# joyecnu/STTODE

Hardware: AMD Instinct MI355X
Metric: predicted-trajectories/sec (20-sample best-of-K) (higher is better)
Workload: dtype f32

## Files before the change

### sttode_amd/csrc/chain.hpp

```cpp
#pragma once
#include <hip/hip_runtime.h>

typedef float f32x4 __attribute__((ext_vector_type(4)));

#define STT_WAVE 64
#define STT_FENCE() asm volatile("" ::: "memory")

__device__ __forceinline__ f32x4 mfma_k16(f32x4 acc, const f32x4 w, const f32x4 b) {
    acc = __builtin_amdgcn_mfma_f32_16x16x4f32(w[0], b[0], acc, 0, 0, 0);
    acc = __builtin_amdgcn_mfma_f32_16x16x4f32(w[1], b[1], acc, 0, 0, 0);
    acc = __builtin_amdgcn_mfma_f32_16x16x4f32(w[2], b[2], acc, 0, 0, 0);
    acc = __builtin_amdgcn_mfma_f32_16x16x4f32(w[3], b[3], acc, 0, 0, 0);
    return acc;
}

__device__ __forceinline__ f32x4 ld4(const float* p) { return *reinterpret_cast<const f32x4*>(p); }
__device__ __forceinline__ void st4(float* p, const f32x4 v) { *reinterpret_cast<f32x4*>(p) = v; }

__device__ __forceinline__ f32x4 relu4(f32x4 v) {
    v[0] = fmaxf(v[0], 0.f); v[1] = fmaxf(v[1], 0.f); v[2] = fmaxf(v[2], 0.f); v[3] = fmaxf(v[3], 0.f);
    return v;
}

__device__ __forceinline__ float sigmoidf_(float x) {
    return __builtin_amdgcn_rcpf(1.0f + __builtin_amdgcn_exp2f(-1.4426950408889634f * x));
}
__device__ __forceinline__ float tanhf_(float x) {
    return 1.0f - 2.0f * __builtin_amdgcn_rcpf(1.0f + __builtin_amdgcn_exp2f(2.8853900817779268f * x));
}
__device__ __forceinline__ float sigmoid_prescaled(float t) { return __builtin_amdgcn_rcpf(1.0f + __builtin_amdgcn_exp2f(t)); }
__device__ __forceinline__ float tanh_prescaled(float t) { return fmaf(-2.0f, __builtin_amdgcn_rcpf(1.0f + __builtin_amdgcn_exp2f(t)), 1.0f); }

__device__ __forceinline__ f32x4 splat4(float v) { f32x4 r = {v, v, v, v}; return r; }

__device__ __forceinline__ float colsum_q(float v) {
    v += __shfl_xor(v, 16, 64);
    v += __shfl_xor(v, 32, 64);
    return v;
}

__device__ __forceinline__ void layernorm64(f32x4 (&x)[4], const float* __restrict__ gamma, const float* __restrict__ beta, int q) {
    float s = 0.f;
#pragma unroll
    for (int T = 0; T < 4; ++T) s += (x[T][0] + x[T][1]) + (x[T][2] + x[T][3]);
    const float mean = colsum_q(s) * (1.0f / 64.0f);
    float v = 0.f;
#pragma unroll
    for (int T = 0; T < 4; ++T)
#pragma unroll
        for (int r = 0; r < 4; ++r) { const float d = x[T][r] - mean; v += d * d; }
    const float rstd = 1.0f / sqrtf(colsum_q(v) * (1.0f / 64.0f) + 1e-5f);
#pragma unroll
    for (int T = 0; T < 4; ++T) {
        const f32x4 g = ld4(gamma + 16 * T + 4 * q), b = ld4(beta + 16 * T + 4 * q);
// ... 27 lines not shown
```

### sttode_amd/csrc/chain32.hip

```cpp
#include "chain.hpp"
#include "latency_bodies.hpp"
#include "frontend_body.hpp"
#include "api_util.hpp"
#include "../../include/sttode_hip.h"
#include <cstdlib>
#include <cstddef>

#ifdef C32_DIAG_TRACE
__shared__ long long g_tr_ph[4];
#define C32_TRACE_BEGIN() long long _tr_t0 = 0, _tr_c0 = 0; if (threadIdx.x == 0 && A.dbg) { _tr_t0 = __builtin_amdgcn_s_memrealtime(); _tr_c0 = __builtin_amdgcn_s_memtime(); }
#define C32_TRACE_END(kind) do { if (threadIdx.x == 0 && A.dbg) { \
        const long long _t1 = __builtin_amdgcn_s_memrealtime(); unsigned _hw, _xcc; \
        asm volatile("s_getreg_b32 %0, hwreg(HW_REG_HW_ID)" : "=s"(_hw)); asm volatile("s_getreg_b32 %0, hwreg(HW_REG_XCC_ID)" : "=s"(_xcc)); \
        const unsigned long long _r = atomicAdd((unsigned long long*)A.dbg, 1ull); if ((long long)_r >= A.dbg[1]) break;  \
        long long* _p = A.dbg + 8 + _r * 12; _p[0] = A.trace_tag; _p[1] = blockIdx.x; _p[2] = (kind); _p[3] = _tr_t0; _p[4] = _t1; _p[5] = _hw; _p[6] = _xcc; \
        _p[8] = g_tr_ph[0]; _p[9] = g_tr_ph[1]; _p[10] = g_tr_ph[2]; _p[7] = __builtin_amdgcn_s_memtime() - _tr_c0; _p[11] = g_tr_ph[3]; } } while (0)
#define C32_TRACE_PHASE(i) do { if (threadIdx.x == 0) g_tr_ph[i] = __builtin_amdgcn_s_memrealtime(); } while (0)
#else
#define C32_TRACE_PHASE(i) do { } while (0)
#define C32_TRACE_BEGIN() do { } while (0)
#define C32_TRACE_END(kind) do { } while (0)
#endif

#include "role_body.hpp"

typedef float f32x16 __attribute__((ext_vector_type(16)));

#ifdef C32_DIAG_NOGATES
#define C32_SIG(x) ((x) * 1e-3f)
#define C32_TANH(x) ((x) * 1e-3f)
#else
#define C32_SIG(x) sigmoid_prescaled(x)
#define C32_TANH(x) tanh_prescaled(x)
#endif

#define C32_TILE 256
#define C32_CMAX 3
#define C32_RING (2 * C32_CMAX * C32_TILE)
#define C32_SLOT 256

struct Role32Args {
    const f32x4* pool; const int2* prog; int prog_len; const float* consts;
    const float* enc_in; const int* last;
    const float* g_in; const float* attn; int ld_attn;
    const float* xpad; int ldx;
    float* pf; float* state0; float* A0x; float* A0y; float* A1y;
    int n, Tp, kte, nwg;
    float ode_time;
    int prio;
    int* counter;
    float* zgen; unsigned zkey0, zkey1; int K;
    const float* past; const int* scene_ptr; int S; float* scene_orig; int* agent_scene;
    float* enc_in_w; float* xpad_w; float* cur_w; float* orig_w; int* last_w;
    float* m_ade; float* m_fde;
};

// ... 14 lines not shown
    int nworkers;
    long long* dbg;
    int trace_tag;
    int xcd_map;
    RoleArgs R;
    Role32Args R32;
};

template <int NY> struct C32Const {
    static constexpr int b2x = 0, b3x = 256, b2y = 288, b3y = 544, gb = 544 + 32 * NY, cb = gb + 384, b2m = cb + 32,
                         b3m = b2m + 256, total = b3m + 32 * NY;
};

__device__ __forceinline__ f32x16 splat16(float v) {
    f32x16 r;
#pragma unroll
    for (int e = 0; e < 16; ++e) r[e] = v;
    return r;
}
__device__ __forceinline__ f32x16 relu16(f32x16 v) {
#pragma unroll
    for (int e = 0; e < 16; ++e) v[e] = fmaxf(v[e], 0.f);
    return v;
}
__device__ __forceinline__ f32x16 ldrows(const float* p, int h) {
    f32x16 r;
#pragma unroll
    for (int a = 0; a < 4; ++a) {
        const f32x4 v = ld4(p + 8 * a + 4 * h);
        r[4 * a + 0] = v[0]; r[4 * a + 1] = v[1]; r[4 * a + 2] = v[2]; r[4 * a + 3] = v[3];
    }
    return r;
}

typedef const __attribute__((address_space(4))) int KProg;

template <int BUF, bool GEN, bool DYN = false>
struct ChainStreamT {
    static constexpr int kBuf = BUF;
    static constexpr int kPieces = (BUF / 64 + 3) / 4, kPairs = (kPieces + 1) / 2;
    const char* pool; KProg* prog; f32x4* ring;
    unsigned ring_addr, loff;
    unsigned qoff, qend;
    int par, lane, wave;
    int2 ld_v, ld_w;
    bool fetched;
// ... 98 lines not shown
        __builtin_amdgcn_sched_barrier(0);
    }
};
typedef ChainStreamT<C32_CMAX * C32_TILE, false> ChainStream;

__device__ __forceinline__ void tile_mma(f32x16& acc, const f32x4* __restrict__ t, const f32x16& B) {
#pragma unroll
    for (int g = 0; g < 4; ++g) {
        const f32x4 a = t[g * 64];
#pragma unroll
        for (int r = 0; r < 4; ++r) acc = __builtin_amdgcn_mfma_f32_32x32x2f32(a[r], B[4 * g + r], acc, 0, 0, 0);
    }
}

__device__ __forceinline__ void gather_rows(const void* base, unsigned voff, unsigned slot_addr) {
    glds16_sv<0>(base, voff, slot_addr);
    glds16_sv<32>(base, voff, slot_addr + 1024);
    glds16_sv<64>(base, voff, slot_addr + 2048);
    glds16_sv<96>(base, voff, slot_addr + 3072);
}
__device__ __forceinline__ unsigned row_off(int row, int width, int h) { return (unsigned)row * (unsigned)(width * 4) + (unsigned)h * 16; }

struct Frag { f32x4 a[4]; };
__device__ __forceinline__ void ldfrag(Frag& f, const f32x4* __restrict__ t) {
#pragma unroll
    for (int g = 0; g < 4; ++g) f.a[g] = t[g * 64];
}
__device__ __forceinline__ void tile_mma2(f32x16& acc, const Frag& cur, const f32x16& B, Frag& nxt, const f32x4* __restrict__ tn) {
#pragma unroll
    for (int g = 0; g < 4; ++g) {
        if (g == 2 && tn) {
            ldfrag(nxt, tn);
            __builtin_amdgcn_sched_barrier(0);
        }
#pragma unroll
        for (int r = 0; r < 4; ++r) acc = __builtin_amdgcn_mfma_f32_32x32x2f32(cur.a[g][r], B[4 * g + r], acc, 0, 0, 0);
    }
}

template <class ST>
__device__ __forceinline__ void tile_mma2f(ST& st, f32x16& acc, const Frag& cur, const f32x16& B, Frag& nxt, const f32x4* __restrict__ tn, int nf = 1) {
#pragma unroll
    for (int g = 0; g < 4; ++g) {
        if (g == 2) {
            __builtin_amdgcn_sched_barrier(0);
            if (nf >= 1) st.fetch();
            if (nf >= 2) st.fetch_more();
            if (tn) ldfrag(nxt, tn);
            __builtin_amdgcn_sched_barrier(0);
        }
#pragma unroll
        for (int r = 0; r < 4; ++r) acc = __builtin_amdgcn_mfma_f32_32x32x2f32(cur.a[g][r], B[4 * g + r], acc, 0, 0, 0);
    }
}

template <int KH, class ST>
__device__ __forceinline__ void mlp_l12(ST& st, const f32x4* slot, const f32x4* zslot, const f32x16* Bh, const float* tab, unsigned aoff,
                                        const float* tab_next, unsigned aoff_next, f32x16 (&acc2)[8], int lane) {
    const unsigned slot_addr = __builtin_amdgcn_readfirstlane(lds_addr(slot));
    constexpr int KT1 = 1 + KH;
    static_assert((KT1 + 8) % 3 == 0, "hidden tile must be a whole number of chunks");
#pragma unroll
    for (int R = 0; R < 8; ++R) acc2[R] = splat16(0.f);
#pragma unroll 1
    for (int ht = 0; ht < 16; ++ht) {
        f32x16 h1, zb;
#pragma unroll
        for (int a = 0; a < 4; ++a) {
            const f32x4 v = slot[a * 64 + lane];
            h1[4 * a + 0] = v[0]; h1[4 * a + 1] = v[1]; h1[4 * a + 2] = v[2]; h1[4 * a + 3] = v[3];
        }
#pragma unroll
        for (int a = 0; a < 4; ++a) {
            const f32x4 v = zslot[a * 64 + lane];
            zb[4 * a + 0] = v[0]; zb[4 * a + 1] = v[1]; zb[4 * a + 2] = v[2]; zb[4 * a + 3] = v[3];
// ... 20 lines not shown
            const f32x4* tn = (i % 3 < 2) ? st.cur() + (i % 3 + 1) * C32_TILE : nullptr;
            if (i == 0) {
                tile_mma2f(st, h1, fr[i & 1], zb, fr[(i + 1) & 1], tn);
            } else if (i < KT1) {
                if (i % 3 == 0) tile_mma2f(st, h1, fr[i & 1], Bh[i - 1], fr[(i + 1) & 1], tn);
                else tile_mma2(h1, fr[i & 1], Bh[i - 1], fr[(i + 1) & 1], tn);
            } else {
                if (i == KT1) h1 = relu16(h1);
                if (i % 3 == 0) tile_mma2f(st, acc2[i - KT1], fr[i & 1], h1, fr[(i + 1) & 1], tn);
                else tile_mma2(acc2[i - KT1], fr[i & 1], h1, fr[(i + 1) & 1], tn);
            }
        }
        st.end();
    }
}

template <int NO, int NEXT = 0, class ST>
__device__ __forceinline__ void mlp_l3(ST& st, f32x16 (&acc2)[8], const float* __restrict__ b2, const float* __restrict__ b3,
                                       f32x16 (&out)[NO], int h) {
#pragma unroll
    for (int R = 0; R < 8; ++R) {
        STT_FENCE();
        const f32x16 b = ldrows(b2 + 32 * R, h);
        acc2[R] = relu16(acc2[R] + b);
        asm volatile("" : "+v"(acc2[R]));
    }
    STT_FENCE();
#pragma unroll
    for (int o = 0; o < NO; ++o) out[o] = ldrows(b3 + 32 * o, h);
    Frag fr[2];
#pragma unroll
    for (int i = 0; i < 8 * NO; ++i) {
        if (i % 3 == 0) {
            if (i > 0) st.end();
            ldfrag(fr[i & 1], st.cur());
            const int left = 8 * NO - (i + 3);
            st.begin(left >= 3 ? 3 : left > 0 ? left : NEXT);
        }
        const f32x4* tn = (i % 3 < 2 && i + 1 < 8 * NO) ? st.cur() + (i % 3 + 1) * C32_TILE : nullptr;
        if (i % 3 == 0) tile_mma2f(st, out[i / 8], fr[i & 1], acc2[i % 8], fr[(i + 1) & 1], tn);
        else tile_mma2(out[i / 8], fr[i & 1], acc2[i % 8], fr[(i + 1) & 1], tn);
    }
    st.end();
}

typedef __bf16 bf16x8 __attribute__((ext_vector_type(8)));
typedef __bf16 bf16x2 __attribute__((ext_vector_type(2)));
// ... 247 lines not shown
            if (g >= g0 && g <= g1) fa.a[g] = tc[g * 64];
        st.begin(3);
#pragma unroll
        for (int g = 0; g < 4; ++g)
            if (g >= g0 && g <= g1)
#pragma unroll
                for (int r = 0; r < 4; ++r) e = __builtin_amdgcn_mfma_f32_32x32x2f32(fa.a[g][r], d[4 * g + r], e, 0, 0, 0);
        __builtin_amdgcn_sched_barrier(0);
        if (pre) st.take_prefetched();
        else st.fetch();
    } else {
        ldfrag(fa, st.cur());
        st.begin(3);
        tile_mma2f(st, e, fa, d, fb, nullptr, pre ? 0 : 1);
        if (pre) st.take_prefetched();
    }
    e = relu16(e);
    st.end();
    return e;
}

template <bool ZS, class ST>
__device__ __forceinline__ void gru32_steps(ST& st, const float* gb, const float* cb, const f32x16& d, f32x16 (&hs)[3], int Tp, int h) {
    if (ZS) {
        const f32x16 e = gru32_conv<ZS>(st, cb, d, 0, Tp, h, false);
        Frag fa, fb;
#pragma unroll
        for (int j = 0; j < 3; ++j) {
            STT_FENCE();
            f32x16 ar = ldrows(gb + 0 * 96 + 32 * j, h);
            ldfrag(fa, st.cur()); st.begin(3);
            tile_mma2f(st, ar, fa, e, fb, nullptr);
            st.end(); ldfrag(fa, st.cur() + 1 * C32_TILE); st.begin(3);
#pragma unroll
            for (int r = 0; r < 16; ++r) ar[r] = C32_SIG(ar[r]);
            STT_FENCE();
            f32x16 az = ldrows(gb + 1 * 96 + 32 * j, h);
            tile_mma2f(st, az, fa, e, fb, nullptr, 2);
            st.end(); st.begin(3);
            st.take_prefetched();
#pragma unroll
            for (int r = 0; r < 16; ++r) az[r] = C32_SIG(az[r]);
            STT_FENCE();
            f32x16 an = ldrows(gb + 3 * 96 + 32 * j, h);
            {
                const f32x16 bi = ldrows(gb + 2 * 96 + 32 * j, h);
#pragma unroll
                for (int r = 0; r < 16; ++r) an[r] = fmaf(ar[r], an[r], bi[r]);
            }
            st.end(); ldfrag(fa, st.cur() + 2 * C32_TILE);
            if (j < 2) st.begin(3); else st.begin();
            STT_FENCE();
            tile_mma2f(st, an, fa, e, fb, nullptr, (j == 2 && 1 < Tp) ? 2 : 1);
            st.end();
#pragma unroll
            for (int r = 0; r < 16; ++r) {
                const float ng = C32_TANH(an[r]);
                hs[j][r] = fmaf(az[r], 0.f - ng, ng);
            }
        }
    }
#pragma unroll 1
    for (int t = ZS ? 1 : 0; t < Tp; ++t) {
        const f32x16 e = gru32_conv<ZS>(st, cb, d, t, Tp, h, ZS);
        Frag fa, fb;
        f32x16 hn[3];
#pragma unroll
        for (int j = 0; j < 3; ++j) {
            STT_FENCE();
            f32x16 ar = ldrows(gb + 0 * 96 + 32 * j, h);
            ldfrag(fa, st.cur()); st.begin(3);
            tile_mma2f(st, ar, fa, e, fb, st.cur() + 1 * C32_TILE);
            tile_mma2(ar, fb, hs[0], fa, st.cur() + 2 * C32_TILE);
            tile_mma2(ar, fa, hs[1], fb, nullptr);
            st.end(); ldfrag(fa, st.cur()); st.begin(3);
            tile_mma2f(st, ar, fa, hs[2], fb, st.cur() + 1 * C32_TILE);
#pragma unroll
            for (int r = 0; r < 16; ++r) ar[r] = C32_SIG(ar[r]);
            STT_FENCE();
            f32x16 az = ldrows(gb + 1 * 96 + 32 * j, h);
            tile_mma2(az, fb, e, fa, st.cur() + 2 * C32_TILE);
            tile_mma2(az, fa, hs[0], fb, nullptr);
            st.end(); ldfrag(fa, st.cur()); st.begin(3);
            tile_mma2f(st, az, fa, hs[1], fb, st.cur() + 1 * C32_TILE);
            tile_mma2(az, fb, hs[2], fa, st.cur() + 2 * C32_TILE);
#pragma unroll
            for (int r = 0; r < 16; ++r) az[r] = C32_SIG(az[r]);
            STT_FENCE();
            f32x16 an = ldrows(gb + 3 * 96 + 32 * j, h);
            tile_mma2(an, fa, hs[0], fb, nullptr);
            st.end(); ldfrag(fa, st.cur());
            if (j < 2) st.begin(3); else st.begin();
            tile_mma2f(st, an, fa, hs[1], fb, st.cur() + 1 * C32_TILE, (ZS && j == 2 && t + 1 < Tp) ? 2 : 1);
            tile_mma2(an, fb, hs[2], fa, st.cur() + 2 * C32_TILE);
            {
                const f32x16 bi = ldrows(gb + 2 * 96 + 32 * j, h);
#pragma unroll
                for (int r = 0; r < 16; ++r) an[r] = fmaf(ar[r], an[r], bi[r]);
            }
            STT_FENCE();
            tile_mma2(an, fa, e, fb, nullptr);
            st.end();
#pragma unroll
            for (int r = 0; r < 16; ++r) {
                const float ng = C32_TANH(an[r]);
                hn[j][r] = fmaf(az[r], hs[j][r] - ng, ng);
            }
        }
#pragma unroll
        for (int j = 0; j < 3; ++j) hs[j] = hn[j];
    }

}

#include "role32.hpp"

__device__ __forceinline__ int opaque(int v) { asm volatile("" : "+v"(v)); return v; }

#ifdef C32_DIAG_STAMPS
#define C32_STAMP(k) do { if (threadIdx.x == 0 && A.dbg && gi < 4) { A.dbg[((size_t)blockIdx.x * 4 + gi) * 16 + 2 * (k)] = __builtin_amdgcn_s_memtime(); \
                                                                    A.dbg[((size_t)blockIdx.x * 4 + gi) * 16 + 2 * (k) + 1] = __builtin_amdgcn_s_memrealtime(); } } while (0)
#else
#define C32_STAMP(k) do { } while (0)
#endif

__host__ __device__ __forceinline__ int fused_block_of(long b, long T, long G, long K, long lead) {
    auto roles_upto = [&](long x) { const long c = (8 * (x + lead + 1) + K - 1) / K; return c < T ? c : T; };
    long lo = -1, hi = G - 1;
    while (lo < hi) {
        const long mid = (lo + hi + 1) >> 1;
        if (mid + roles_upto(mid) <= b) lo = mid; else hi = mid - 1;
    }
    if (lo >= 0 && lo + roles_upto(lo) == b) return (int)lo;
    return -1 - (int)(b - (lo + 1));
}

__host__ __device__ __forceinline__ int xcd_group(int b, int G) {
    const int x = b & 7, i = b >> 3, q = G >> 3, r = G & 7;
    return x * q + (x < r ? x : r) + i;
}

template <int NY, int FUSE, bool B3M, bool ZS>
__global__ __launch_bounds__(256, 2) void traj_chain_kernel(ChainArgs A) {
    constexpr bool kDynCount = !B3M && ((NY == 1 && FUSE == 2 && !ZS) || (NY == 2 && FUSE == 1 && ZS));
    typedef ChainStreamT<B3M ? C32_BUF_B3 : C32_CMAX * C32_TILE, B3M, kDynCount> Stream;
    extern __shared__ __attribute__((aligned(16))) char smem[];
    f32x4* ring = reinterpret_cast<f32x4*>(smem);
    f32x4* slots = ring + 2 * Stream::kBuf;
    f32x4* zslots = slots + 4 * C32_SLOT;
    float* cst = reinterpret_cast<float*>(zslots + 4 * C32_SLOT);
    int* sq = reinterpret_cast<int*>(cst + C32Const<NY>::total);
    typedef C32Const<NY> CO;

    const int lane = threadIdx.x & 63, c = lane & 31, h = lane >> 5;
    const int wave = __builtin_amdgcn_readfirstlane(threadIdx.x >> 6);
    const f32x4* slot = slots + wave * C32_SLOT;
    const f32x4* zslot = zslots + wave * C32_SLOT;
    const unsigned slot_addr = __builtin_amdgcn_readfirstlane(lds_addr(slot));
    const unsigned zslot_addr = __builtin_amdgcn_readfirstlane(lds_addr(zslot));
    const int ngroups = (A.ncols + 127) >> 7;

    C32_TRACE_BEGIN();
    if (FUSE == 2 && (int)blockIdx.x < A.R32.nwg) {
        role32_body<ZS>(*(KRole32Args*)((const __attribute__((address_space(4))) char*)__builtin_amdgcn_kernarg_segment_ptr() + offsetof(ChainArgs, R32)),
                    blockIdx.x, smem);
        C32_TRACE_END(1);
        return;
// ... 59 lines not shown
            sq[1] = (FUSE == 2 && A.persistent && ngroups > A.nworkers) ? A.nworkers + atomicAdd(A.counter, 1)
                    : (FUSE == 0 && A.persistent) ? atomicAdd(A.counter, 1) : ngroups;

        f32x16 acc2[8];
        f32x16 d;
        {
            agent = opaque(agent);
            f32x16 xo[1];
            const unsigned ao = row_off(agent, 512, h);
            if (B3M) {
                mlp_l12_b3<0, true>(st, slot, zslot, nullptr, A.A0x, ao, A.A0y, ao, acc2, lane);
                mlp_l3_b3<1>(st, acc2, cst + CO::b2x, cst + CO::b3x, xo, h);
            } else {
                mlp_l12<0>(st, slot, zslot, nullptr, A.A0x, ao, A.A0y, ao, acc2, lane);
                mlp_l3<1, 3>(st, acc2, cst + CO::b2x, cst + CO::b3x, xo, h);
            }
            agent = opaque(agent);
            const float* xp = A.xpad + (size_t)agent * A.ldx;
#pragma unroll
            for (int a = 0; a < 4; ++a) {
                f32x4 v = splat4(0.f);
                if (8 * a + 4 * h < A.ldx) v = ld4(xp + 8 * a + 4 * h);
#pragma unroll
                for (int b = 0; b < 4; ++b) d[4 * a + b] = v[b] - xo[0][4 * a + b];
            }
        }
        STT_FENCE();
        C32_STAMP(1);
        {
            agent = opaque(agent);
            f32x16 yo[NY];
            const unsigned ao = row_off(agent, 512, h);
            if (B3M) {
                mlp_l12_b3<0, true>(st, slot, zslot, nullptr, A.A0y, ao, A.A1y, ao, acc2, lane);
                mlp_l3_b3<NY>(st, acc2, cst + CO::b2y, cst + CO::b3y, yo, h);
            } else {
                mlp_l12<0>(st, slot, zslot, nullptr, A.A0y, ao, A.A1y, ao, acc2, lane);
                mlp_l3<NY, 1>(st, acc2, cst + CO::b2y, cst + CO::b3y, yo, h);
            }
            if (live) {
                float* prow = A.park + (size_t)opaque(col) * A.Tf2;
#pragma unroll
                for (int o = 0; o < NY; ++o)
#pragma unroll
                    for (int a = 0; a < 4; ++a) {
                        const int row0 = 32 * o + 8 * a + 4 * h;
                        float* p = prow + row0;
// ... 33 lines not shown
            {
                agent = opaque(agent);
                const float cx = A.cur[2 * agent], cy = A.cur[2 * agent + 1];
                const float ox = A.orig[2 * agent], oy = A.orig[2 * agent + 1];
                const bool vec = (A.Tf2 & 3) == 0;
                const float* yrow = A.park + (size_t)opaque(colc) * A.Tf2;
                float* prow = A.pred + (size_t)opaque(col) * A.Tf2;
                const float* grow = FUSE == 2 && A.m_gt ? A.m_gt + (size_t)agent * A.Tf2 : nullptr;
                float dd[NY][4][2];
#pragma unroll
                for (int o = 0; o < NY; ++o)
#pragma unroll
                    for (int a = 0; a < 4; ++a) {
                        const int row0 = 32 * o + 8 * a + 4 * h;
                        const bool whole = vec && row0 + 3 < A.Tf2;
                        f32x4 y0 = splat4(0.f);
                        if (whole) y0 = ld4(yrow + row0);
                        else {
#pragma unroll
                            for (int b = 0; b < 4; ++b)
                                if (row0 + b < A.Tf2) y0[b] = yrow[row0 + b];
                        }
                        f32x4 v;
                        v[0] = ((y0[0] + yo[o][4 * a + 0]) + cx) + ox;
                        v[1] = ((y0[1] + yo[o][4 * a + 1]) + cy) + oy;
                        v[2] = ((y0[2] + yo[o][4 * a + 2]) + cx) + ox;
                        v[3] = ((y0[3] + yo[o][4 * a + 3]) + cy) + oy;
                        if (live) {
                            if (whole) st4(prow + row0, v);
                            else {
#pragma unroll
                                for (int b = 0; b < 4; ++b)
                                    if (row0 + b < A.Tf2) prow[row0 + b] = v[b];
                            }
                        }
                        dd[o][a][0] = dd[o][a][1] = 0.f;
                        if (FUSE == 2 && grow) {
                            if (row0 < A.Tf2) { const float2 g = *reinterpret_cast<const float2*>(grow + row0); dd[o][a][0] = bok_dist(v[0], v[1], g.x, g.y, A.m_scale); }
                            if (row0 + 2 < A.Tf2) { const float2 g = *reinterpret_cast<const float2*>(grow + row0 + 2); dd[o][a][1] = bok_dist(v[2], v[3], g.x, g.y, A.m_scale); }
                        }
                    }
                if (FUSE == 2 && grow) {
                    const int Tf = A.Tf2 >> 1;
                    float acc = 0.f, fdl = -1.f;
#pragma unroll
                    for (int o = 0; o < NY; ++o)
#pragma unroll
                        for (int a = 0; a < 4; ++a) {
                            const int t0 = (32 * o + 8 * a + 4 * h) >> 1;
                            float mine = acc;
// ... 381 lines not shown
```

### sttode_amd/csrc/frontend_body.hpp

```cpp
#pragma once
#include <hip/hip_runtime.h>

template <bool SC1> __device__ __forceinline__ void fe_store(float* p, float v) {
    if (SC1) __hip_atomic_store(p, v, __ATOMIC_RELAXED, __HIP_MEMORY_SCOPE_AGENT);
    else *p = v;
}

template <bool SC1, int TMAX = 0>
__device__ __forceinline__ void agent_inputs_core(int a, const float* __restrict__ seq, int T, int TPX, int vel_from_norm, float ox, float oy,
                                                  int last, const float* __restrict__ prev_last,
                                                  float* __restrict__ xpad, float* __restrict__ enc_in, float* __restrict__ cur,
                                                  float* __restrict__ orig, int* __restrict__ last_flag,
                                                  const float2* __restrict__ preloaded = nullptr) {
    const float* p = seq + (size_t)a * T * 2;
    float* xp = xpad ? xpad + (size_t)a * 16 * TPX : nullptr;
    float pnx = 0.f, pny = 0.f, pwx = 0.f, pwy = 0.f;
    const bool have_prev = prev_last != nullptr;
    if (have_prev) {
        pwx = prev_last[2 * a];
        pwy = prev_last[2 * a + 1];
        pnx = pwx - ox;
        pny = pwy - oy;
    }
    float2 wb[TMAX > 0 ? TMAX : 1];
    if (TMAX > 0) {
#pragma unroll
        for (int t = 0; t < TMAX; ++t)
            if (t < T) wb[t] = preloaded ? preloaded[t] : reinterpret_cast<const float2*>(p)[t];
    }
#pragma unroll
    for (int t = 0; t < (TMAX > 0 ? TMAX : T); ++t) {
        if (TMAX > 0 && t >= T) continue;
        const float wx = TMAX > 0 ? wb[t].x : p[2 * t], wy = TMAX > 0 ? wb[t].y : p[2 * t + 1];
        const float nx = wx - ox, ny = wy - oy;
        float vx, vy;
        if (t == 0 && !have_prev) {
            const float w1x = TMAX > 0 ? wb[1 < TMAX ? 1 : 0].x : p[2], w1y = TMAX > 0 ? wb[1 < TMAX ? 1 : 0].y : p[3];
            if (vel_from_norm) { vx = (w1x - ox) - nx; vy = (w1y - oy) - ny; }
            else { vx = w1x - wx; vy = w1y - wy; }
        } else {
            if (vel_from_norm) { vx = nx - pnx; vy = ny - pny; }
            else { vx = wx - pwx; vy = wy - pwy; }
        }
        if (enc_in) {
            float* e = enc_in + ((size_t)a * T + t) * 4;
            e[0] = nx; e[1] = ny; e[2] = vx; e[3] = vy;
        }
        if (xp) { fe_store<SC1>(xp + 2 * t, nx); fe_store<SC1>(xp + 2 * t + 1, ny); }
        pnx = nx; pny = ny; pwx = wx; pwy = wy;
    }
    if (xp)
        for (int k = 2 * T; k < 16 * TPX; ++k) fe_store<SC1>(xp + k, 0.f);
    if (cur) { fe_store<SC1>(cur + 2 * a, pnx); fe_store<SC1>(cur + 2 * a + 1, pny); }
    if (orig) { fe_store<SC1>(orig + 2 * a, ox); fe_store<SC1>(orig + 2 * a + 1, oy); }
    if (last_flag) last_flag[a] = last;
}

__device__ __forceinline__ float bok_dist(float px, float py, float gx, float gy, float scale) {
    const float dx = (px - gx) * scale, dy = (py - gy) * scale;
    return sqrtf(__fmaf_rn(dx, dx, dy * dy));
}
```

### sttode_amd/csrc/role32.hpp

```cpp
#pragma once

struct R32C {
    static constexpr int bc = 0, wlast = 64, bi = 128, bg = 192, ln1w = 256, ln1b = 320, l1b = 384, l2b = 1408, ln2w = 1472, ln2b = 1536,
                         gb = 1600, cb = 1984, b1x = 2016, b1y = 2528, b11 = 3040, total = 3552;
};

typedef const __attribute__((address_space(4))) Role32Args KRole32Args;

template <class ST> struct TileFeed {
    ST& st; int t, cnt; bool pre;
    Frag cur, nxt;
    __device__ __forceinline__ explicit TileFeed(ST& s) : st(s), t(0), cnt(0), pre(false) {}
    __device__ __forceinline__ void open() {
        cnt = st.cnt;
        t = 0;
        ldfrag(cur, st.cur());
        st.begin();
        pre = false;
    }
    __device__ __forceinline__ void mma(f32x16& acc, const f32x16& B) {
        if (t == cnt) { st.end(true); open(); }
        else if (pre) cur = nxt;
        const f32x4* tn = t + 1 < cnt ? st.cur() + (t + 1) * C32_TILE : nullptr;
        tile_mma2f(st, acc, cur, B, nxt, tn, t == 0 ? 1 : 0);
        pre = tn != nullptr;
        ++t;
    }
    __device__ __forceinline__ void close() { st.end(true); }
};

__device__ __forceinline__ float halfsum32(float v) { return v + __shfl_xor(v, 32, 64); }

__device__ __forceinline__ void layernorm64_c32(f32x16 (&x)[2], const float* gamma, const float* beta, int h) {
    float s = 0.f;
#pragma unroll
    for (int j = 0; j < 2; ++j)
#pragma unroll
        for (int r = 0; r < 16; r += 4) s += (x[j][r] + x[j][r + 1]) + (x[j][r + 2] + x[j][r + 3]);
    const float mean = halfsum32(s) * (1.0f / 64.0f);
    float v = 0.f;
#pragma unroll
    for (int j = 0; j < 2; ++j)
#pragma unroll
        for (int r = 0; r < 16; ++r) { const float dd = x[j][r] - mean; v += dd * dd; }
    const float rstd = 1.0f / sqrtf(halfsum32(v) * (1.0f / 64.0f) + 1e-5f);
#pragma unroll
    for (int j = 0; j < 2; ++j) {
        const f32x16 g = ldrows(gamma + 32 * j, h), b = ldrows(beta + 32 * j, h);
#pragma unroll
        for (int r = 0; r < 16; ++r) x[j][r] = (x[j][r] - mean) * rstd * g[r] + b[r];
    }
}

__device__ __forceinline__ void strows(float* p, const f32x16& v, int h) {
#pragma unroll
    for (int a = 0; a < 4; ++a) {
        const f32x4 w = {v[4 * a], v[4 * a + 1], v[4 * a + 2], v[4 * a + 3]};
        st4(p + 8 * a + 4 * h, w);
    }
}

template <int KT, class FD>
__device__ __forceinline__ void table32(FD& fd, const float* bias, float* out, const f32x16 (&B)[7], int col, bool live, int h) {
#pragma unroll 1
    for (int rt = 0; rt < 16; ++rt) {
        f32x16 acc = ldrows(bias + 32 * rt, h);
#pragma unroll
        for (int kt = 0; kt < KT; ++kt) fd.mma(acc, B[kt]);
        if (live) strows(out + (size_t)col * 512 + 32 * rt, acc, h);
    }
}

__device__ __forceinline__ void philox4x32_10(unsigned (&c)[4], unsigned k0, unsigned k1) {
// ... 1 lines not shown
    for (int r = 0; r < 10; ++r) {
        const unsigned long long p0 = (unsigned long long)0xD2511F53u * c[0], p1 = (unsigned long long)0xCD9E8D57u * c[2];
        const unsigned n0 = (unsigned)(p1 >> 32) ^ c[1] ^ k0, n2 = (unsigned)(p0 >> 32) ^ c[3] ^ k1;
        c[0] = n0; c[1] = (unsigned)p1; c[2] = n2; c[3] = (unsigned)p0;
        k0 += 0x9E3779B9u; k1 += 0xBB67AE85u;
    }
}
__device__ __forceinline__ void latents32(float* z, unsigned k0, unsigned k1, int wg, int n, int K) {
    const int a0 = wg * 128, na = n - a0 < 128 ? n - a0 : 128;
    const long first4 = (long)a0 * K * 8;
    const int count4 = na * K * 8;
    for (int i = threadIdx.x; i < count4; i += blockDim.x) {
        const unsigned long long g4 = (unsigned long long)(first4 + i);
        unsigned c[4] = {(unsigned)g4, (unsigned)(g4 >> 32), 0u, 0u};
        philox4x32_10(c, k0, k1);
        f32x4 v;
#pragma unroll
        for (int p = 0; p < 2; ++p) {
            const float u1 = (float)(c[2 * p] >> 8) * 5.9604644775390625e-8f + 2.98023223876953125e-8f;
            const float u2 = (float)(c[2 * p + 1] >> 8) * 5.9604644775390625e-8f + 2.98023223876953125e-8f;
            const float rad = sqrtf(-2.0f * __logf(u1));
            float sn, cs;
            __sincosf(6.283185307179586f * u2, &sn, &cs);
            v[2 * p] = rad * cs; v[2 * p + 1] = rad * sn;
        }
        st4(z + (first4 + i) * 4, v);
    }
}

__device__ __forceinline__ void frontend32(KRole32Args& R, int wg) {
    const int a = wg * 128 + (int)threadIdx.x;
    if (threadIdx.x < 128 && a < R.n) {
        int lo = 0, hi = R.S - 1;
        while (lo < hi) {
            const int mid = (lo + hi + 1) >> 1;
            if (R.scene_ptr[mid] <= a) lo = mid; else hi = mid - 1;
        }
        const int a0 = R.scene_ptr[lo], a1 = R.scene_ptr[lo + 1];
        float sx = 0.f, sy = 0.f;
        for (int aa = a0; aa < a1; ++aa) {
            sx += R.past[((size_t)aa * R.Tp + (R.Tp - 1)) * 2 + 0];
            sy += R.past[((size_t)aa * R.Tp + (R.Tp - 1)) * 2 + 1];
        }
        const float inv = (float)(a1 - a0);
        const float ox = sx / inv, oy = sy / inv;
        if (a == a0) { R.scene_orig[2 * lo] = ox; R.scene_orig[2 * lo + 1] = oy; }
        R.agent_scene[a] = lo;
        agent_inputs_core<false, 16>(a, R.past, R.Tp, R.ldx / 16, 1, ox, oy, a == a1 - 1, nullptr, R.xpad_w, R.enc_in_w, R.cur_w, R.orig_w, R.last_w);
    }
}

template <bool ZS>
__device__ __forceinline__ void role32_body(KRole32Args& R, int wg, char* smem) {
    f32x4* ring = reinterpret_cast<f32x4*>(smem);
    float* cst = reinterpret_cast<float*>(ring + C32_RING);
    const int lane = threadIdx.x & 63, c = lane & 31, h = lane >> 5;
    const int wave = __builtin_amdgcn_readfirstlane(threadIdx.x >> 6);
    if (R.prio > 0) __builtin_amdgcn_s_setprio(3);
    if (wg == 0 && threadIdx.x == 0) *R.counter = 0;
    if (R.m_ade && threadIdx.x < 128 && wg * 128 + (int)threadIdx.x < R.n) {
        R.m_ade[wg * 128 + threadIdx.x] = INFINITY;
        R.m_fde[wg * 128 + threadIdx.x] = INFINITY;
    }
    if (R.past) frontend32(R, wg);
    if (R.zgen) latents32(R.zgen, R.zkey0, R.zkey1, wg, R.n, R.K);
// ... 33 lines not shown
        for (int j = 0; j < 3; ++j) strows(R.state0 + (size_t)col * 96 + 32 * j, hs[j], h);
    }
    STT_FENCE();
    TileFeed<ChainStream> fd(st);
    fd.open();
    f32x16 G[2], S[2];
    if (R.attn == nullptr) {
        f32x16 X[2];
        const float* ep = R.enc_in + (size_t)colc * (4 * R.Tp);
#pragma unroll
        for (int kt = 0; kt < 2; ++kt)
#pragma unroll
            for (int a = 0; a < 4; ++a) {
                f32x4 v = splat4(0.f);
                if (32 * kt + 8 * a + 4 * h < 4 * R.Tp) v = ld4(ep + 32 * kt + 8 * a + 4 * h);
#pragma unroll
                for (int b = 0; b < 4; ++b) X[kt][4 * a + b] = v[b];
            }
        const float lastf = R.last[colc] ? 1.0f : 0.0f;
#pragma unroll
        for (int j = 0; j < 2; ++j) {
            const f32x16 b = ldrows(cst + R32C::bc + 32 * j, h), wl = ldrows(cst + R32C::wlast + 32 * j, h);
#pragma unroll
            for (int r = 0; r < 16; ++r) G[j][r] = fmaf(wl[r], lastf, b[r]);
            fd.mma(G[j], X[0]);
            if (R.kte > 1) fd.mma(G[j], X[1]);
        }
        S[0] = G[0]; S[1] = G[1];
    } else {
#pragma unroll
        for (int j = 0; j < 2; ++j) {
            G[j] = ldrows(R.g_in + (size_t)colc * 64 + 32 * j, h);
            S[j] = ldrows(R.attn + (size_t)colc * R.ld_attn + 32 * j, h);
        }
    }
    f32x16 XR[2];
#pragma unroll
    for (int j = 0; j < 2; ++j) {
        f32x16 vi = ldrows(cst + R32C::bi + 32 * j, h);
        fd.mma(vi, S[0]);
        fd.mma(vi, S[1]);
        f32x16 vg = ldrows(cst + R32C::bg + 32 * j, h);
        fd.mma(vg, S[0]);
        fd.mma(vg, S[1]);
#pragma unroll
        for (int r = 0; r < 16; ++r) XR[j][r] = G[j][r] + tanhf(vi[r]) * sigmoidf_(vg[r]);
    }
    layernorm64_c32(XR, cst + R32C::ln1w, cst + R32C::ln1b, h);
    {
        f32x16 FF[2];
        FF[0] = splat16(0.f); FF[1] = splat16(0.f);
#pragma unroll 1
        for (int ht = 0; ht < 32; ++ht) {
            f32x16 hid = ldrows(cst + R32C::l1b + 32 * ht, h);
            fd.mma(hid, XR[0]);
            fd.mma(hid, XR[1]);
            hid = relu16(hid);
            fd.mma(FF[0], hid);
            fd.mma(FF[1], hid);
        }
#pragma unroll
        for (int j = 0; j < 2; ++j) {
            const f32x16 b = ldrows(cst + R32C::l2b + 32 * j, h);
            XR[j] = XR[j] + (FF[j] + b);
        }
    }
    layernorm64_c32(XR, cst + R32C::ln2w, cst + R32C::ln2b, h);
    f32x16 B7[7];
#pragma unroll
    for (int j = 0; j < 2; ++j) {
        B7[j] = G[j];
        B7[2 + j] = relu16(G[j] + XR[j] * R.ode_time);
    }
#pragma unroll
    for (int j = 0; j < 3; ++j) B7[4 + j] = hs[j];
    if (live) {
#pragma unroll
        for (int j = 0; j < 4; ++j) strows(R.pf + (size_t)col * 128 + 32 * j, B7[j], h);
    }
    table32<7>(fd, cst + R32C::b1x, R.A0x, B7, col, live, h);
    table32<7>(fd, cst + R32C::b1y, R.A0y, B7, col, live, h);
    table32<4>(fd, cst + R32C::b11, R.A1y, B7, col, live, h);
    fd.close();
}

struct QNet32Args {
    const f32x4* pool; const int2* prog; int prog_len; const float* bias;
    const float* pf; float* z; const float* eps;
    int n, K, h1t, h2t, eps_mode;
};

__device__ __forceinline__ f32x16 tanh16(f32x16 v) {
#pragma unroll
    for (int e = 0; e < 16; ++e) v[e] = tanhf(v[e]);
    return v;
// ... 53 lines not shown
```

Measured before the change: 86.75 million.

## Interleave GRU gate activations between MFMA instructions to hide transcendental latency

The sigmoid and tanh gate activations in the 32-wide GRU steps are moved out of separate loops and spread one element at a time between individual MFMA instructions via fill callbacks bracketed by sched_barriers. The tanh/hidden update of each block is deferred into the next block's MFMA chain. Many arithmetic ops are additionally pinned with empty asm constraints to fix evaluation order and stop the compiler from reassociating or fusing them. This aims to overlap VALU/transcendental work with matrix-core latency, at the cost of more rigid scheduling, extra live registers, and some changed rounding from new fmaf use.

```diff
diff --git a/sttode_amd/csrc/chain.hpp b/sttode_amd/csrc/chain.hpp
--- a/sttode_amd/csrc/chain.hpp
+++ b/sttode_amd/csrc/chain.hpp
@@ -30,6 +30,12 @@
 }
 __device__ __forceinline__ float sigmoid_prescaled(float t) { return __builtin_amdgcn_rcpf(1.0f + __builtin_amdgcn_exp2f(t)); }
 __device__ __forceinline__ float tanh_prescaled(float t) { return fmaf(-2.0f, __builtin_amdgcn_rcpf(1.0f + __builtin_amdgcn_exp2f(t)), 1.0f); }
+
+__device__ __forceinline__ float pin1(float x) { asm volatile("" : "+v"(x)); return x; }
+__device__ __forceinline__ float sigmoid_prescaled_el(float t) { return pin1(__builtin_amdgcn_rcpf(pin1(1.0f + __builtin_amdgcn_exp2f(t)))); }
+__device__ __forceinline__ float tanh_prescaled_el(float t) {
+    return pin1(fmaf(-2.0f, __builtin_amdgcn_rcpf(pin1(1.0f + __builtin_amdgcn_exp2f(t))), 1.0f));
+}
 
 __device__ __forceinline__ f32x4 splat4(float v) { f32x4 r = {v, v, v, v}; return r; }
 
diff --git a/sttode_amd/csrc/chain32.hip b/sttode_amd/csrc/chain32.hip
--- a/sttode_amd/csrc/chain32.hip
+++ b/sttode_amd/csrc/chain32.hip
@@ -29,9 +29,13 @@
 #ifdef C32_DIAG_NOGATES
 #define C32_SIG(x) ((x) * 1e-3f)
 #define C32_TANH(x) ((x) * 1e-3f)
+#define C32_SIG1(x) pin1((x) * 1e-3f)
+#define C32_TANH1(x) pin1((x) * 1e-3f)
 #else
 #define C32_SIG(x) sigmoid_prescaled(x)
 #define C32_TANH(x) tanh_prescaled(x)
+#define C32_SIG1(x) sigmoid_prescaled_el(x)
+#define C32_TANH1(x) tanh_prescaled_el(x)
 #endif
 
 #define C32_TILE 256
@@ -92,6 +96,16 @@
 #pragma unroll
     for (int e = 0; e < 16; ++e) v[e] = fmaxf(v[e], 0.f);
     return v;
+}
+__device__ __forceinline__ f32x16 add16(f32x16 a, const f32x16& b) {
+#pragma unroll
+    for (int e = 0; e < 16; ++e) a[e] = pin1(a[e] + b[e]);
+    return a;
+}
+__device__ __forceinline__ f32x16 relu_add16(f32x16 a, const f32x16& b) {
+#pragma unroll
+    for (int e = 0; e < 16; ++e) a[e] = pin1(fmaxf(a[e] + b[e], 0.f));
+    return a;
 }
 __device__ __forceinline__ f32x16 ldrows(const float* p, int h) {
     f32x16 r;
@@ -236,11 +250,17 @@
 __device__ __forceinline__ unsigned row_off(int row, int width, int h) { return (unsigned)row * (unsigned)(width * 4) + (unsigned)h * 16; }
 
 struct Frag { f32x4 a[4]; };
+struct NoFill { __device__ __forceinline__ void operator()(int) const {} };
+template <class F> struct IsFill { static constexpr bool value = true; };
+template <> struct IsFill<NoFill> { static constexpr bool value = false; };
+template <class E> __device__ __forceinline__ void fill_2tiles(int tile, int k, E&& el) { if ((k & 1) == 0) el(8 * tile + (k >> 1)); }
+template <class E> __device__ __forceinline__ void fill_1tile(int k, E&& el) { if (k < 15) el(k); if (k == 14) el(15); }
 __device__ __forceinline__ void ldfrag(Frag& f, const f32x4* __restrict__ t) {
 #pragma unroll
     for (int g = 0; g < 4; ++g) f.a[g] = t[g * 64];
 }
-__device__ __forceinline__ void tile_mma2(f32x16& acc, const Frag& cur, const f32x16& B, Frag& nxt, const f32x4* __restrict__ tn) {
+template <class F = NoFill>
+__device__ __forceinline__ void tile_mma2(f32x16& acc, const Frag& cur, const f32x16& B, Frag& nxt, const f32x4* __restrict__ tn, F fill = F()) {
 #pragma unroll
     for (int g = 0; g < 4; ++g) {
         if (g == 2 && tn) {
@@ -248,12 +268,20 @@
             __builtin_amdgcn_sched_barrier(0);
         }
 #pragma unroll
-        for (int r = 0; r < 4; ++r) acc = __builtin_amdgcn_mfma_f32_32x32x2f32(cur.a[g][r], B[4 * g + r], acc, 0, 0, 0);
-    }
-}
-
-template <class ST>
-__device__ __forceinline__ void tile_mma2f(ST& st, f32x16& acc, const Frag& cur, const f32x16& B, Frag& nxt, const f32x4* __restrict__ tn, int nf = 1) {
+        for (int r = 0; r < 4; ++r) {
+            acc = __builtin_amdgcn_mfma_f32_32x32x2f32(cur.a[g][r], B[4 * g + r], acc, 0, 0, 0);
+            if (IsFill<F>::value) {
+                __builtin_amdgcn_sched_barrier(0);
+                fill(4 * g + r);
+                __builtin_amdgcn_sched_barrier(0);
+            }
+        }
+    }
+}
+
+template <class ST, class F = NoFill>
+__device__ __forceinline__ void tile_mma2f(ST& st, f32x16& acc, const Frag& cur, const f32x16& B, Frag& nxt, const f32x4* __restrict__ tn, int nf = 1,
+                                           F fill = F()) {
 #pragma unroll
     for (int g = 0; g < 4; ++g) {
         if (g == 2) {
@@ -264,7 +292,14 @@
             __builtin_amdgcn_sched_barrier(0);
         }
 #pragma unroll
-        for (int r = 0; r < 4; ++r) acc = __builtin_amdgcn_mfma_f32_32x32x2f32(cur.a[g][r], B[4 * g + r], acc, 0, 0, 0);
+        for (int r = 0; r < 4; ++r) {
+            acc = __builtin_amdgcn_mfma_f32_32x32x2f32(cur.a[g][r], B[4 * g + r], acc, 0, 0, 0);
+            if (IsFill<F>::value) {
+                __builtin_amdgcn_sched_barrier(0);
+                fill(4 * g + r);
+                __builtin_amdgcn_sched_barrier(0);
+            }
+        }
     }
 }
 
@@ -331,7 +366,7 @@
     for (int R = 0; R < 8; ++R) {
         STT_FENCE();
         const f32x16 b = ldrows(b2 + 32 * R, h);
-        acc2[R] = relu16(acc2[R] + b);
+        acc2[R] = relu_add16(acc2[R], b);
         asm volatile("" : "+v"(acc2[R]));
     }
     STT_FENCE();
@@ -625,42 +660,44 @@
 
 template <bool ZS, class ST>
 __device__ __forceinline__ void gru32_steps(ST& st, const float* gb, const float* cb, const f32x16& d, f32x16 (&hs)[3], int Tp, int h) {
+    constexpr bool ROT = ZS;
+    f32x16 pn, pz;
     if (ZS) {
         const f32x16 e = gru32_conv<ZS>(st, cb, d, 0, Tp, h, false);
         Frag fa, fb;
+        hs[2] = splat16(0.f);
 #pragma unroll
         for (int j = 0; j < 3; ++j) {
+            auto tanh_prev = [&](int i) __attribute__((always_inline)) {
+                const float ng = C32_TANH1(pn[i]);
+                hs[(j + 2) % 3][i] = pin1(fmaf(pz[i], pin1(0.f - ng), ng));
+            };
             STT_FENCE();
             f32x16 ar = ldrows(gb + 0 * 96 + 32 * j, h);
             ldfrag(fa, st.cur()); st.begin(3);
-            tile_mma2f(st, ar, fa, e, fb, nullptr);
+            if (j > 0) tile_mma2f(st, ar, fa, e, fb, nullptr, 1, [&](int k) __attribute__((always_inline)) { fill_1tile(k, tanh_prev); });
+            else tile_mma2f(st, ar, fa, e, fb, nullptr);
             st.end(); ldfrag(fa, st.cur() + 1 * C32_TILE); st.begin(3);
-#pragma unroll
-            for (int r = 0; r < 16; ++r) ar[r] = C32_SIG(ar[r]);
             STT_FENCE();
             f32x16 az = ldrows(gb + 1 * 96 + 32 * j, h);
-            tile_mma2f(st, az, fa, e, fb, nullptr, 2);
+            tile_mma2f(st, az, fa, e, fb, nullptr, 2,
+                       [&](int k) __attribute__((always_inline)) { fill_1tile(k, [&](int i) __attribute__((always_inline)) { ar[i] = C32_SIG1(ar[i]); }); });
             st.end(); st.begin(3);
             st.take_prefetched();
-#pragma unroll
-            for (int r = 0; r < 16; ++r) az[r] = C32_SIG(az[r]);
             STT_FENCE();
             f32x16 an = ldrows(gb + 3 * 96 + 32 * j, h);
             {
                 const f32x16 bi = ldrows(gb + 2 * 96 + 32 * j, h);
 #pragma unroll
-                for (int r = 0; r < 16; ++r) an[r] = fmaf(ar[r], an[r], bi[r]);
+                for (int r = 0; r < 16; ++r) an[r] = pin1(fmaf(ar[r], an[r], bi[r]));
             }
             st.end(); ldfrag(fa, st.cur() + 2 * C32_TILE);
             if (j < 2) st.begin(3); else st.begin();
             STT_FENCE();
-            tile_mma2f(st, an, fa, e, fb, nullptr, (j == 2 && 1 < Tp) ? 2 : 1);
+            tile_mma2f(st, an, fa, e, fb, nullptr, (j == 2 && 1 < Tp) ? 2 : 1,
+                       [&](int k) __attribute__((always_inline)) { fill_1tile(k, [&](int i) __attribute__((always_inline)) { az[i] = C32_SIG1(az[i]); }); });
             st.end();
-#pragma unroll
-            for (int r = 0; r < 16; ++r) {
-                const float ng = C32_TANH(an[r]);
-                hs[j][r] = fmaf(az[r], 0.f - ng, ng);
-            }
+            pn = an; pz = az;
         }
     }
 #pragma unroll 1
@@ -670,50 +707,68 @@
         f32x16 hn[3];
 #pragma unroll
         for (int j = 0; j < 3; ++j) {
+            auto tanh_prev = [&](int i) __attribute__((always_inline)) {
+                const float ng = C32_TANH1(pn[i]);
+                const float hv = pin1(fmaf(pz[i], pin1(hs[(j + 2) % 3][i] - ng), ng));
+                if (j > 0) hn[j - 1 + (j == 0)][i] = hv; else hs[2][i] = hv;
+            };
             STT_FENCE();
             f32x16 ar = ldrows(gb + 0 * 96 + 32 * j, h);
             ldfrag(fa, st.cur()); st.begin(3);
-            tile_mma2f(st, ar, fa, e, fb, st.cur() + 1 * C32_TILE);
-            tile_mma2(ar, fb, hs[0], fa, st.cur() + 2 * C32_TILE);
+            if (j > 0 || ROT) {
+                tile_mma2f(st, ar, fa, e, fb, st.cur() + 1 * C32_TILE, 1, [&](int k) __attribute__((always_inline)) { fill_2tiles(0, k, tanh_prev); });
+                tile_mma2(ar, fb, hs[0], fa, st.cur() + 2 * C32_TILE, [&](int k) __attribute__((always_inline)) { fill_2tiles(1, k, tanh_prev); });
+            } else {
+                tile_mma2f(st, ar, fa, e, fb, st.cur() + 1 * C32_TILE);
+                tile_mma2(ar, fb, hs[0], fa, st.cur() + 2 * C32_TILE);
+            }
             tile_mma2(ar, fa, hs[1], fb, nullptr);
             st.end(); ldfrag(fa, st.cur()); st.begin(3);
             tile_mma2f(st, ar, fa, hs[2], fb, st.cur() + 1 * C32_TILE);
-#pragma unroll
-            for (int r = 0; r < 16; ++r) ar[r] = C32_SIG(ar[r]);
             STT_FENCE();
             f32x16 az = ldrows(gb + 1 * 96 + 32 * j, h);
-            tile_mma2(az, fb, e, fa, st.cur() + 2 * C32_TILE);
-            tile_mma2(az, fa, hs[0], fb, nullptr);
+            auto sig_ar = [&](int i) __attribute__((always_inline)) { ar[i] = C32_SIG1(ar[i]); };
+            tile_mma2(az, fb, e, fa, st.cur() + 2 * C32_TILE, [&](int k) __attribute__((always_inline)) { fill_2tiles(0, k, sig_ar); });
+            tile_mma2(az, fa, hs[0], fb, nullptr, [&](int k) __attribute__((always_inline)) { fill_2tiles(1, k, sig_ar); });
             st.end(); ldfrag(fa, st.cur()); st.begin(3);
             tile_mma2f(st, az, fa, hs[1], fb, st.cur() + 1 * C32_TILE);
             tile_mma2(az, fb, hs[2], fa, st.cur() + 2 * C32_TILE);
-#pragma unroll
-            for (int r = 0; r < 16; ++r) az[r] = C32_SIG(az[r]);
             STT_FENCE();
             f32x16 an = ldrows(gb + 3 * 96 + 32 * j, h);
             tile_mma2(an, fa, hs[0], fb, nullptr);
             st.end(); ldfrag(fa, st.cur());
             if (j < 2) st.begin(3); else st.begin();
-            tile_mma2f(st, an, fa, hs[1], fb, st.cur() + 1 * C32_TILE, (ZS && j == 2 && t + 1 < Tp) ? 2 : 1);
-            tile_mma2(an, fb, hs[2], fa, st.cur() + 2 * C32_TILE);
+            auto sig_az = [&](int i) __attribute__((always_inline)) { az[i] = C32_SIG1(az[i]); };
+            tile_mma2f(st, an, fa, hs[1], fb, st.cur() + 1 * C32_TILE, (ZS && j == 2 && t + 1 < Tp) ? 2 : 1,
+                       [&](int k) __attribute__((always_inline)) { fill_2tiles(0, k, sig_az); });
+            tile_mma2(an, fb, hs[2], fa, st.cur() + 2 * C32_TILE, [&](int k) __attribute__((always_inline)) { fill_2tiles(1, k, sig_az); });
             {
                 const f32x16 bi = ldrows(gb + 2 * 96 + 32 * j, h);
 #pragma unroll
-                for (int r = 0; r < 16; ++r) an[r] = fmaf(ar[r], an[r], bi[r]);
+                for (int r = 0; r < 16; ++r) an[r] = pin1(fmaf(ar[r], an[r], bi[r]));
             }
             STT_FENCE();
             tile_mma2(an, fa, e, fb, nullptr);
             st.end();
+            pn = an; pz = az;
+        }
+        if (!ROT) {
 #pragma unroll
             for (int r = 0; r < 16; ++r) {
-                const float ng = C32_TANH(an[r]);
-                hn[j][r] = fmaf(az[r], hs[j][r] - ng, ng);
-            }
-        }
-#pragma unroll
-        for (int j = 0; j < 3; ++j) hs[j] = hn[j];
-    }
-
+                const float ng = C32_TANH1(pn[r]);
+                hn[2][r] = pin1(fmaf(pz[r], pin1(hs[2][r] - ng), ng));
+            }
+        }
+#pragma unroll
+        for (int j = 0; j < (ROT ? 2 : 3); ++j) hs[j] = hn[j];
+    }
+    if (ROT) {
+#pragma unroll
+        for (int r = 0; r < 16; ++r) {
+            const float ng = C32_TANH1(pn[r]);
+            hs[2][r] = pin1(fmaf(pz[r], pin1(hs[2][r] - ng), ng));
+        }
+    }
 }
 
 #include "role32.hpp"
@@ -746,6 +801,7 @@
 template <int NY, int FUSE, bool B3M, bool ZS>
 __global__ __launch_bounds__(256, 2) void traj_chain_kernel(ChainArgs A) {
     constexpr bool kDynCount = !B3M && ((NY == 1 && FUSE == 2 && !ZS) || (NY == 2 && FUSE == 1 && ZS));
+    constexpr bool kPinD = NY == 3;
     typedef ChainStreamT<B3M ? C32_BUF_B3 : C32_CMAX * C32_TILE, B3M, kDynCount> Stream;
     extern __shared__ __attribute__((aligned(16))) char smem[];
     f32x4* ring = reinterpret_cast<f32x4*>(smem);
@@ -851,7 +907,10 @@
                 f32x4 v = splat4(0.f);
                 if (8 * a + 4 * h < A.ldx) v = ld4(xp + 8 * a + 4 * h);
 #pragma unroll
-                for (int b = 0; b < 4; ++b) d[4 * a + b] = v[b] - xo[0][4 * a + b];
+                for (int b = 0; b < 4; ++b) {
+                    d[4 * a + b] = v[b] - xo[0][4 * a + b];
+                    if (kPinD) d[4 * a + b] = pin1(d[4 * a + b]);
+                }
             }
         }
         STT_FENCE();
@@ -931,10 +990,9 @@
                                 if (row0 + b < A.Tf2) y0[b] = yrow[row0 + b];
                         }
                         f32x4 v;
-                        v[0] = ((y0[0] + yo[o][4 * a + 0]) + cx) + ox;
-                        v[1] = ((y0[1] + yo[o][4 * a + 1]) + cy) + oy;
-                        v[2] = ((y0[2] + yo[o][4 * a + 2]) + cx) + ox;
-                        v[3] = ((y0[3] + yo[o][4 * a + 3]) + cy) + oy;
+#pragma unroll
+                        for (int b = 0; b < 4; ++b)
+                            v[b] = pin1(pin1(pin1(y0[b] + yo[o][4 * a + b]) + ((b & 1) ? cy : cx)) + ((b & 1) ? oy : ox));
                         if (live) {
                             if (whole) st4(prow + row0, v);
                             else {
diff --git a/sttode_amd/csrc/frontend_body.hpp b/sttode_amd/csrc/frontend_body.hpp
--- a/sttode_amd/csrc/frontend_body.hpp
+++ b/sttode_amd/csrc/frontend_body.hpp
@@ -1,5 +1,12 @@
 #pragma once
 #include <hip/hip_runtime.h>
+
+template <bool PIN> __device__ __forceinline__ float fe_sub(float a, float b) {
+    if (PIN) asm volatile("" : "+v"(a));
+    float r = a - b;
+    if (PIN) asm volatile("" : "+v"(r));
+    return r;
+}
 
 template <bool SC1> __device__ __forceinline__ void fe_store(float* p, float v) {
     if (SC1) __hip_atomic_store(p, v, __ATOMIC_RELAXED, __HIP_MEMORY_SCOPE_AGENT);
@@ -12,6 +19,7 @@
                                                   float* __restrict__ xpad, float* __restrict__ enc_in, float* __restrict__ cur,
                                                   float* __restrict__ orig, int* __restrict__ last_flag,
                                                   const float2* __restrict__ preloaded = nullptr) {
+    constexpr bool P = TMAX > 0;
     const float* p = seq + (size_t)a * T * 2;
     float* xp = xpad ? xpad + (size_t)a * 16 * TPX : nullptr;
     float pnx = 0.f, pny = 0.f, pwx = 0.f, pwy = 0.f;
@@ -19,8 +27,8 @@
     if (have_prev) {
         pwx = prev_last[2 * a];
         pwy = prev_last[2 * a + 1];
-        pnx = pwx - ox;
-        pny = pwy - oy;
+        pnx = fe_sub<P>(pwx, ox);
+        pny = fe_sub<P>(pwy, oy);
     }
     float2 wb[TMAX > 0 ? TMAX : 1];
     if (TMAX > 0) {
@@ -32,15 +40,15 @@
     for (int t = 0; t < (TMAX > 0 ? TMAX : T); ++t) {
         if (TMAX > 0 && t >= T) continue;
         const float wx = TMAX > 0 ? wb[t].x : p[2 * t], wy = TMAX > 0 ? wb[t].y : p[2 * t + 1];
-        const float nx = wx - ox, ny = wy - oy;
+        const float nx = fe_sub<P>(wx, ox), ny = fe_sub<P>(wy, oy);
         float vx, vy;
         if (t == 0 && !have_prev) {
             const float w1x = TMAX > 0 ? wb[1 < TMAX ? 1 : 0].x : p[2], w1y = TMAX > 0 ? wb[1 < TMAX ? 1 : 0].y : p[3];
-            if (vel_from_norm) { vx = (w1x - ox) - nx; vy = (w1y - oy) - ny; }
-            else { vx = w1x - wx; vy = w1y - wy; }
+            if (vel_from_norm) { vx = fe_sub<P>(fe_sub<P>(w1x, ox), nx); vy = fe_sub<P>(fe_sub<P>(w1y, oy), ny); }
+            else { vx = fe_sub<P>(w1x, wx); vy = fe_sub<P>(w1y, wy); }
         } else {
-            if (vel_from_norm) { vx = nx - pnx; vy = ny - pny; }
-            else { vx = wx - pwx; vy = wy - pwy; }
+            if (vel_from_norm) { vx = fe_sub<P>(nx, pnx); vy = fe_sub<P>(ny, pny); }
+            else { vx = fe_sub<P>(wx, pwx); vy = fe_sub<P>(wy, pwy); }
         }
         if (enc_in) {
             float* e = enc_in + ((size_t)a * T + t) * 4;
diff --git a/sttode_amd/csrc/role32.hpp b/sttode_amd/csrc/role32.hpp
--- a/sttode_amd/csrc/role32.hpp
+++ b/sttode_amd/csrc/role32.hpp
@@ -36,19 +36,19 @@
 #pragma unroll
     for (int j = 0; j < 2; ++j)
 #pragma unroll
-        for (int r = 0; r < 16; r += 4) s += (x[j][r] + x[j][r + 1]) + (x[j][r + 2] + x[j][r + 3]);
-    const float mean = halfsum32(s) * (1.0f / 64.0f);
+        for (int r = 0; r < 16; r += 4) s = pin1(s + pin1(pin1(x[j][r] + x[j][r + 1]) + pin1(x[j][r + 2] + x[j][r + 3])));
+    const float mean = pin1(halfsum32(s) * (1.0f / 64.0f));
     float v = 0.f;
 #pragma unroll
     for (int j = 0; j < 2; ++j)
 #pragma unroll
-        for (int r = 0; r < 16; ++r) { const float dd = x[j][r] - mean; v += dd * dd; }
+        for (int r = 0; r < 16; ++r) { const float dd = pin1(x[j][r] - mean); v = pin1(v + pin1(dd * dd)); }
     const float rstd = 1.0f / sqrtf(halfsum32(v) * (1.0f / 64.0f) + 1e-5f);
 #pragma unroll
     for (int j = 0; j < 2; ++j) {
         const f32x16 g = ldrows(gamma + 32 * j, h), b = ldrows(beta + 32 * j, h);
 #pragma unroll
-        for (int r = 0; r < 16; ++r) x[j][r] = (x[j][r] - mean) * rstd * g[r] + b[r];
+        for (int r = 0; r < 16; ++r) x[j][r] = pin1(fmaf(pin1(pin1(x[j][r] - mean) * rstd), g[r], b[r]));
     }
 }
 
@@ -96,7 +96,7 @@
             const float rad = sqrtf(-2.0f * __logf(u1));
             float sn, cs;
             __sincosf(6.283185307179586f * u2, &sn, &cs);
-            v[2 * p] = rad * cs; v[2 * p + 1] = rad * sn;
+            v[2 * p] = pin1(rad * cs); v[2 * p + 1] = pin1(rad * sn);
         }
         st4(z + (first4 + i) * 4, v);
     }
@@ -113,8 +113,8 @@
         const int a0 = R.scene_ptr[lo], a1 = R.scene_ptr[lo + 1];
         float sx = 0.f, sy = 0.f;
         for (int aa = a0; aa < a1; ++aa) {
-            sx += R.past[((size_t)aa * R.Tp + (R.Tp - 1)) * 2 + 0];
-            sy += R.past[((size_t)aa * R.Tp + (R.Tp - 1)) * 2 + 1];
+            sx = pin1(sx + R.past[((size_t)aa * R.Tp + (R.Tp - 1)) * 2 + 0]);
+            sy = pin1(sy + R.past[((size_t)aa * R.Tp + (R.Tp - 1)) * 2 + 1]);
         }
         const float inv = (float)(a1 - a0);
         const float ox = sx / inv, oy = sy / inv;
@@ -194,7 +194,7 @@
         for (int j = 0; j < 2; ++j) {
             const f32x16 b = ldrows(cst + R32C::bc + 32 * j, h), wl = ldrows(cst + R32C::wlast + 32 * j, h);
 #pragma unroll
-            for (int r = 0; r < 16; ++r) G[j][r] = fmaf(wl[r], lastf, b[r]);
+            for (int r = 0; r < 16; ++r) G[j][r] = pin1(fmaf(wl[r], lastf, b[r]));
             fd.mma(G[j], X[0]);
             if (R.kte > 1) fd.mma(G[j], X[1]);
         }
@@ -216,7 +216,10 @@
         fd.mma(vg, S[0]);
         fd.mma(vg, S[1]);
 #pragma unroll
-        for (int r = 0; r < 16; ++r) XR[j][r] = G[j][r] + tanhf(vi[r]) * sigmoidf_(vg[r]);
+        for (int r = 0; r < 16; ++r) {
+            const float ti = tanhf(vi[r]), sg = sigmoidf_(vg[r]);
+            XR[j][r] = (j == 1 && r == 15) ? pin1(G[j][r] + pin1(ti * sg)) : pin1(fmaf(ti, sg, G[j][r]));
+        }
     }
     layernorm64_c32(XR, cst + R32C::ln1w, cst + R32C::ln1b, h);
     {
@@ -234,7 +237,7 @@
 #pragma unroll
         for (int j = 0; j < 2; ++j) {
             const f32x16 b = ldrows(cst + R32C::l2b + 32 * j, h);
-            XR[j] = XR[j] + (FF[j] + b);
+            XR[j] = add16(XR[j], add16(FF[j], b));
         }
     }
     layernorm64_c32(XR, cst + R32C::ln2w, cst + R32C::ln2b, h);
@@ -242,7 +245,9 @@
 #pragma unroll
     for (int j = 0; j < 2; ++j) {
         B7[j] = G[j];
-        B7[2 + j] = relu16(G[j] + XR[j] * R.ode_time);
+#pragma unroll
+        for (int r = 0; r < 16; ++r)
+            B7[2 + j][r] = pin1(fmaxf(fmaf(XR[j][r], R.ode_time, G[j][r]), 0.f));
     }
 #pragma unroll
     for (int j = 0; j < 3; ++j) B7[4 + j] = hs[j];
```

After: 85.70 million. -1.2%, worse.
